# SunBangjie/FYP-BidirectionalPathTracer

Measured on AMD Instinct MI355X. Metric: Mrays/s + RMSE vs the scalar oracle, BDPT pass, Sponza-class scene 1920x1080 depth 8, higher is better.
Workload: dtype f32

## Files before the change

fyp-bidirectionalpathtracer_amd/__init__.py:

```python
import ctypes as C

from . import abi, tiling
from .abi import (Camera, Counters, GBuffer, GBufferParams, Params, SceneDesc, Stripes, Tile, TileInfo, load_library)

__all__ = ["abi", "tiling", "Scene", "Context", "FramePipeline", "load_library", "source_hash", "ADAPTIVE_DEFAULTS",
           "adaptive_params"]

GBUFFER_CHANNELS = ("WorldPosition", "WorldNormal", "MaterialDiffuse", "MaterialSpecRough", "MaterialExtraParams",
                    "Emissive")
OUTPUT_CHANNEL = "PipelineOutput"


class BdptError(RuntimeError):
    pass


def source_hash():
    import glob
    import hashlib
    import os
    here = os.path.dirname(os.path.abspath(__file__))
    root = os.path.dirname(here)
    files = sorted(glob.glob(os.path.join(here, "csrc", "*.hip")) + glob.glob(os.path.join(here, "csrc", "*.hpp")) +
                   glob.glob(os.path.join(here, "csrc", "*.h")) + glob.glob(os.path.join(here, "csrc", "*.cpp")) +
# ... 465 lines not shown
    def sync(self, stream=None):
        self._check(self._lib.bdpt_sync(self._h, stream), "bdpt_sync")

    def test_rng(self, val0, val1, draws):
        import numpy as np
        val0 = np.ascontiguousarray(val0, np.uint32)
        val1 = np.ascontiguousarray(val1, np.uint32)
        n = val0.size
        st = np.zeros((n, draws), np.uint32)
        fl = np.zeros((n, draws), np.float32)
        self._check(self._lib.bdpt_test_rng(self._h, val0.ctypes.data, val1.ctypes.data, n, draws, st.ctypes.data,
                                            fl.ctypes.data), "bdpt_test_rng")
        return st, fl

    def test_trace(self, rays, mode):
        import numpy as np
        rays = np.ascontiguousarray(rays, np.float32).reshape(-1, 8)
        n = rays.shape[0]
        prim = np.zeros(n, np.int32)
        tuv = np.zeros((n, 3), np.float32)
        self._check(self._lib.bdpt_test_trace(self._h, rays.ctypes.data, n, mode, prim.ctypes.data, tuv.ctypes.data),
                    "bdpt_test_trace")
        return prim, tuv

    def test_trace_shadow(self, rays):
        import numpy as np
        rays = np.ascontiguousarray(rays, np.float32)
        n = rays.shape[0]
        vis = np.zeros(n, np.uint8)
        deep = C.c_uint32(0)
        self._check(self._lib.bdpt_test_trace_shadow(self._h, rays.ctypes.data, n, vis.ctypes.data, C.byref(deep)),
                    "bdpt_test_trace_shadow")
        return vis, deep.value

    def test_bsdf(self, recs, mat_index):
        import numpy as np
        recs = np.ascontiguousarray(recs, np.float32).reshape(-1, 20)
        out = np.zeros((recs.shape[0], 16), np.float32)
        self._check(self._lib.bdpt_test_bsdf(self._h, recs.ctypes.data, recs.shape[0], mat_index, out.ctypes.data),
                    "bdpt_test_bsdf")
        return out

    def area_light_info(self):
        info = abi.AreaLightInfo()
        self._check(self._lib.bdpt_get_area_light_info(self._h, C.byref(info)), "bdpt_get_area_light_info")
        return info

    def test_area_light_sample(self, mode, states, points=None):
        import numpy as np
        states = np.ascontiguousarray(states, np.uint32).reshape(-1)
        n = states.shape[0]
        pts = None
        if points is not None:
            pts = np.ascontiguousarray(points, np.float32).reshape(n, 3)
        out = np.zeros((n, 16), np.float32)
        self._check(self._lib.bdpt_test_area_light_sample(self._h, mode, states.ctypes.data,
                                                          None if pts is None else pts.ctypes.data, n, out.ctypes.data),
                    "bdpt_test_area_light_sample")
        return out

    def close(self):
        if self._h:
            self._lib.bdpt_destroy(self._h)
            self._h = None

    def __del__(self):
# ... 217 lines not shown
```

fyp-bidirectionalpathtracer_amd/abi.py:

```python
import ctypes as C
import os

_HERE = os.path.dirname(os.path.abspath(__file__))
LIB_PATH = os.path.join(_HERE, "csrc", "libbdpt_amd.so")

BDPT_MAX_DEPTH = 16
BDPT_MAX_LIGHTS = 16
PARAM_COUNTERS = 1
PARAM_DEFER_RESOLVE = 2
PARAM_NO_NEE = 4
PARAM_NO_SPLAT = 8
PARAM_NO_CONNECT = 16
PARAM_SPECULAR_FROM_LOBE = 32
PARAM_MIS_POWER = 64
PARAM_MIS_LINEAR = 128
PARAM_DEFER_TAIL = 256
PARAM_KEEP_COUNTERS = 512
PARAM_ENV_ON_MISS = 1024
PARAM_EMISSIVE_HITS = 2048
PARAM_AREA_LIGHTS = 4096
PREPARE_PRIMARY = 1
PREPARE_BMFR = 2
PREPARE_REFIT = 4
PREPARE_LIGHT_GROUPS = 8
# ... 195 lines not shown
    "bdpt_adaptive_reset": (C.c_int, [C.c_void_p, C.POINTER(AdaptiveState), C.c_void_p]),
    "bdpt_adaptive_update": (C.c_int, [C.c_void_p, C.POINTER(AdaptiveParams), C.POINTER(AdaptiveState), C.c_void_p, C.c_void_p]),
    "bdpt_prepare": (C.c_int, [C.c_void_p, C.c_uint32]),
    "bdpt_resize_stripes": (C.c_int, [C.c_void_p, C.c_uint32, C.c_uint32, Stripes, C.c_uint32]),
    "bdpt_stripe_rows": (C.c_uint32, [C.c_uint32, C.c_uint32]),
    "bdpt_get_tile_info": (C.c_int, [C.c_void_p, C.POINTER(TileInfo)]),
    "bdpt_tile_row_ranges": (C.c_int, [C.c_void_p, C.POINTER(C.c_uint32), C.c_uint32]),
    "bdpt_resolve_tile": (C.c_int, [C.c_void_p, C.c_void_p, C.c_void_p, C.c_void_p]),
    "bdpt_accumulate_tile": (C.c_int, [C.c_void_p, C.c_void_p, C.c_void_p, C.c_uint32, C.c_uint32, C.c_void_p]),
    "bdpt_test_tree_builder": (C.c_int, [C.c_int]),
    "bdpt_bvh_recs_hash": (C.c_int, [C.POINTER(SceneDesc), C.c_int, C.POINTER(C.c_uint64), C.POINTER(BvhInfo)]),
    "bdpt_bvh_build_hash": (C.c_int, [C.POINTER(SceneDesc), C.c_int, C.POINTER(C.c_uint64), C.POINTER(BvhInfo)]),
    "bdpt_splat_buffer": (C.c_int, [C.c_void_p, C.POINTER(C.c_void_p), C.POINTER(C.c_uint64)]),
    "bdpt_set_splat_buffer": (C.c_int, [C.c_void_p, C.c_void_p, C.c_uint64]),
    "bdpt_resolve": (C.c_int, [C.c_void_p, C.c_void_p, C.c_uint32, C.c_void_p, C.c_void_p]),
    "bdpt_bmfr_execute": (C.c_int, [C.c_void_p, C.POINTER(BmfrParams), C.POINTER(GBuffer), C.c_void_p, C.c_void_p]),
    "bdpt_bmfr_reset": (C.c_int, [C.c_void_p]),
    "bdpt_bmfr_history_bytes": (C.c_int, [C.c_void_p, C.POINTER(C.c_uint64)]),
    "bdpt_bmfr_save_history": (C.c_int, [C.c_void_p, C.c_void_p, C.c_uint64]),
    "bdpt_bmfr_load_history": (C.c_int, [C.c_void_p, C.c_void_p, C.c_uint64]),
    "bdpt_tile_pack": (C.c_int, [C.c_void_p, C.c_void_p, C.c_void_p, C.c_uint32, C.c_void_p]),
    "bdpt_tile_unpack": (C.c_int, [C.c_void_p, C.c_uint32, C.c_void_p, C.c_void_p, C.c_uint32, C.c_void_p]),
    "bdpt_camera_view_proj": (C.c_int, [C.POINTER(C.c_float), C.POINTER(C.c_float), C.POINTER(C.c_float), C.c_float,
                                        C.c_float, C.c_float, C.c_float, C.c_float, C.POINTER(C.c_float)]),
    "bdpt_accumulate": (C.c_int, [C.c_void_p, C.c_void_p, C.c_void_p, C.c_uint32, C.c_uint32, C.c_uint64,
                                  C.c_void_p]),
    "bdpt_get_counters": (C.c_int, [C.c_void_p, C.POINTER(Counters)]),
    "bdpt_get_stage_times": (C.c_int, [C.c_void_p, C.POINTER(C.c_char_p), C.POINTER(C.c_float), C.c_int]),
    "bdpt_enable_stage_timing": (C.c_int, [C.c_void_p, C.c_int]),
    "bdpt_sync": (C.c_int, [C.c_void_p, C.c_void_p]),
    "bdpt_test_rng": (C.c_int, [C.c_void_p, C.c_void_p, C.c_void_p, C.c_uint32, C.c_uint32, C.c_void_p, C.c_void_p]),
    "bdpt_test_trace": (C.c_int, [C.c_void_p, C.c_void_p, C.c_uint32, C.c_int, C.c_void_p, C.c_void_p]),
    "bdpt_test_trace_shadow": (C.c_int, [C.c_void_p, C.c_void_p, C.c_uint32, C.c_void_p, C.c_void_p]),
    "bdpt_test_bsdf": (C.c_int, [C.c_void_p, C.c_void_p, C.c_uint32, C.c_uint32, C.c_void_p]),
    "bdpt_get_area_light_info": (C.c_int, [C.c_void_p, C.POINTER(AreaLightInfo)]),
    "bdpt_test_area_light_sample": (C.c_int, [C.c_void_p, C.c_uint32, C.c_void_p, C.c_void_p, C.c_uint32, C.c_void_p]),
    "bdpt_scene_create_cornell": (C.c_void_p, []),
    "bdpt_scene_create_atrium": (C.c_void_p, [C.c_uint32, C.c_uint32]),
    "bdpt_scene_create_atrium_uneven": (C.c_void_p, [C.c_uint32, C.c_uint32]),
    "bdpt_scene_create_courtyard": (C.c_void_p, [C.c_uint32, C.c_uint32, C.c_float]),
    "bdpt_scene_create_soup": (C.c_void_p, [C.c_uint32, C.c_uint32, C.c_float]),
    "bdpt_scene_load": (C.c_void_p, [C.c_char_p, C.c_char_p, C.c_uint32]),
    "bdpt_scene_load_threads": (C.c_int, [C.c_int]),
    "bdpt_scene_destroy": (None, [C.c_void_p]),
    "bdpt_image_load": (C.c_int, [C.c_char_p, C.POINTER(C.c_uint32), C.POINTER(C.c_uint32), C.POINTER(C.c_uint32), C.c_void_p, C.c_uint64,
                                  C.c_char_p, C.c_uint32]),
    "bdpt_image_load_hdr": (C.c_int, [C.c_char_p, C.POINTER(C.c_uint32), C.POINTER(C.c_uint32), C.c_void_p, C.c_uint64, C.c_char_p, C.c_uint32]),
    "bdpt_scene_get_desc": (C.c_int, [C.c_void_p, C.POINTER(SceneDesc)]),
    "bdpt_scene_get_camera": (C.c_int, [C.c_void_p, C.c_float, C.POINTER(Camera)]),
}

_lib = None


def load_library(path=None):
    global _lib
    if _lib is not None and path is None:
        return _lib
    p = path or LIB_PATH
    if not os.path.exists(p):
        raise RuntimeError(
            f"{p} not found: the HIP extension is not built (run __graft_entry__.build()). "
            "There is no CPU fallback for the render pass.")
    lib = C.CDLL(p, mode=C.RTLD_GLOBAL)
    for name, (res, args) in PROTOTYPES.items():
        fn = getattr(lib, name)
# ... 6 lines not shown
```

fyp-bidirectionalpathtracer_amd/csrc/api.cpp:

```cpp
#include <hip/hip_runtime.h>

#include <cmath>
#include <cstdio>
#include <cstdlib>
#include <cstring>
#include <future>
#include <functional>
#include <atomic>
#include <chrono>
#include <string>
#include <thread>
#include <vector>

#include "../../include/bdpt.h"
#include <new>

#include "bvh.h"
#include "kernels.h"
#include "refit.h"
#include "scene_bvh.h"

using namespace bdpt;

namespace {
// ... 1881 lines not shown
    out_info->numAlwaysPass = sb.numAlwaysPass;
  }
  return BDPT_OK;
} catch (const std::bad_alloc&) {
  return BDPT_E_NOMEM;
} catch (...) {
  return BDPT_E_INVALID;
}

int bdpt_get_counters(bdpt_ctx* c, bdpt_counters* out) {
  if (!c || !out) return BDPT_E_INVALID;
  if (!c->haveSize) return BDPT_E_STATE;
  ENTER(c);
  HIPCHK(c, hipStreamSynchronize(c->lastStream));
  DevCounters h;
  HIPCHK(c, hipMemcpy(&h, c->counters, sizeof(h), hipMemcpyDeviceToHost));
  static_assert(sizeof(bdpt_counters) == 17 * sizeof(uint64_t), "counter fields");
  uint64_t* o = reinterpret_cast<uint64_t*>(out);
  for (int f = 0; f < 13; f++) {
    o[f] = 0;
    for (uint32_t sh = 0; sh < kCounterShards; sh++) o[f] += h.v[sh][f];
  }
  out->alphaTestsClosest = out->alphaTestsShadow = out->hintedNee = out->hintedSplat = 0;
  for (uint32_t sh = 0; sh < kCounterShards; sh++) {
    out->alphaTestsClosest += h.v[sh][C_ALPHA_CLOSEST];
    out->alphaTestsShadow += h.v[sh][C_ALPHA_SHADOW];
    out->hintedNee += h.v[sh][C_HINT_NEE];
    out->hintedSplat += h.v[sh][C_HINT_SPLAT];
  }
  out->raysPrimary = (uint64_t)c->P.Np;
  return BDPT_OK;
}

int bdpt_enable_stage_timing(bdpt_ctx* c, int enable) {
  if (!c) return BDPT_E_INVALID;
  c->timing = enable != 0;
  return BDPT_OK;
}

int bdpt_get_stage_times(bdpt_ctx* c, const char** names, float* ms, int cap) {
  if (!c || !names || !ms) return BDPT_E_INVALID;
  if (!c->timing || c->numStages == 0) return 0;
  ENTER(c);
  HIPCHK(c, hipEventSynchronize(c->ev[c->numStages]));
  int n = std::min(cap, c->numStages);
  for (int i = 0; i < n; i++) {
    names[i] = c->stageNames[i];
    float t = 0.0f;
    HIPCHK(c, hipEventElapsedTime(&t, c->ev[i], c->ev[i + 1]));
    ms[i] = t;
  }
  for (int i = 0; i < c->numSideStages && n < cap; i++, n++) {
    names[n] = c->sideNames[i];
    float t = 0.0f;
    HIPCHK(c, hipEventElapsedTime(&t, c->sideEv[2 * i], c->sideEv[2 * i + 1]));
    ms[n] = t;
  }
  return n;
}

int bdpt_sync(bdpt_ctx* c, void* stream) {
  if (!c) return BDPT_E_INVALID;
  ENTER(c);
  HIPCHK(c, hipStreamSynchronize(reinterpret_cast<hipStream_t>(stream)));
  return BDPT_OK;
}
// ... 173 lines not shown
```

fyp-bidirectionalpathtracer_amd/csrc/device_trace.hpp:

```cpp
#pragma once
#include "bvh.h"
#include "device_scene.hpp"

namespace bdpt {
#define BD __device__ __forceinline__
#define BDPT_ONE_WAVE_PER_GROUP()               \
  do {                                          \
    if (blockDim.x != (unsigned)kWave) return;  \
  } while (0)

struct Hit {
  int prim;
  float t, u, v;
  uint32_t rec;
};

constexpr int kDone = (int)0x80000000;

struct TravState {
  f3 o, d, idir;
  uint32_t neg;
  float tmin, tmax;
  int cur, sp;
  Hit best;
};

BD float clampedRcp(float d) {
  float r = 1.0f / d;
  if (!(fabsf(r) <= 1.0e30f)) r = copysignf(1.0e30f, d);
  return r;
}

BD void travInit(TravState& T, f3 o, f3 d, float tmin, float tmax) {
  T.o = o;
  T.d = d;
  T.idir = mk(clampedRcp(d.x), clampedRcp(d.y), clampedRcp(d.z));
  T.neg = (d.x < 0.0f ? 1u : 0u) | (d.y < 0.0f ? 2u : 0u) | (d.z < 0.0f ? 4u : 0u);
  T.tmin = tmin;
  T.tmax = tmax;
  T.sp = 0;
  T.best.prim = -1;
  T.best.t = tmax;
  T.best.u = 0.0f;
  T.best.v = 0.0f;
  T.best.rec = 0xFFFFFFFFu;
  const bool finite = (o.x == o.x) && (o.y == o.y) && (o.z == o.z) && (d.x == d.x) && (d.y == d.y) && (d.z == d.z);
  T.cur = (finite && (tmax > tmin)) ? 0 : kDone;
}

template <int KL>
BD int* ovfSlot(const SceneDev& S, int e) {
  return S.stackOvf + (size_t)(e - KL) * S.stackOvfStride + (size_t)blockIdx.x * kWave + (threadIdx.x & 63u);
}
template <int KL>
BD void stackStore(const SceneDev& S, int* stk, int e, int ref) {
  if (KL < kStackEntries && e >= KL)
    *ovfSlot<KL>(S, e) = ref;
  else
    stk[e * kWave] = ref;
}
template <int KL>
BD int travPop(const SceneDev& S, TravState& T, const int* stk) {
  if (T.sp == 0) return kDone;
  T.sp--;
  if (KL < kStackEntries && T.sp >= KL) return *ovfSlot<KL>(S, T.sp);
  return stk[T.sp * kWave];
}
template <int KL>
BD void travPush(const SceneDev& S, TravState& T, int* stk, int ref) {
  stackStore<KL>(S, stk, T.sp, ref);
  T.sp++;
}

BD float ubyte(uint32_t w, int c) { return (float)((w >> (8 * c)) & 0xffu); }

template <int ORDER, int KL = kStackEntries>
BD void nodeStep(const SceneDev& S, TravState& T, int* stk) {
  const uint4* np = S.recs + (size_t)T.cur * kRecF4;
  const uint4 q0 = np[0], q1 = np[1], q2 = np[2];
  const float sx = __uint_as_float((q0.w << 23) & 0x7f800000u), sy = __uint_as_float((q0.w << 15) & 0x7f800000u),
              sz = __uint_as_float((q0.w << 7) & 0x7f800000u);
  const float ax = sx * T.idir.x, ay = sy * T.idir.y, az = sz * T.idir.z;
  const float bx = (__uint_as_float(q0.x) - T.o.x) * T.idir.x, by = (__uint_as_float(q0.y) - T.o.y) * T.idir.y,
              bz = (__uint_as_float(q0.z) - T.o.z) * T.idir.z;
// ... 388 lines not shown
```

fyp-bidirectionalpathtracer_amd/csrc/kernels.h:

```cpp
#pragma once
#include <hip/hip_runtime.h>
#include <stdint.h>

#include "../../include/bdpt.h"
#include "texture_planes.h"

namespace bdpt {

constexpr int kWave = 64;
#ifndef KSTACK
#define KSTACK 32
#endif
constexpr int kStackEntries = KSTACK;
#ifndef BDPT_STACK_LDS
#define BDPT_STACK_LDS 24
#endif
constexpr int kStackLds = BDPT_STACK_LDS < KSTACK ? BDPT_STACK_LDS : KSTACK;
constexpr int kMaxPersistentPerCU = 32;
constexpr int kStackOvfRows = KSTACK - kStackLds;
constexpr int kShadeRecF4 = 7;
constexpr uint32_t kNoRay = 0xFFFFFFFFu;
constexpr uint32_t kNumSubQueues = 32;
#ifndef BDPT_FETCH_CHUNK
#define BDPT_FETCH_CHUNK 256
#endif
constexpr uint32_t kFetchChunk = BDPT_FETCH_CHUNK;
constexpr uint32_t kCursorStride = 32;
constexpr uint32_t kCursorBlock = kNumSubQueues * kCursorStride;
#ifndef BDPT_RAY_SUBQUEUES
#define BDPT_RAY_SUBQUEUES 32
#endif
constexpr uint32_t kNumRaySubQueues = BDPT_RAY_SUBQUEUES;
constexpr uint32_t kRayCursorBlock = kNumRaySubQueues * kCursorStride;
constexpr uint32_t kCounterShards = 64;

enum : int { F_COL = 0, F_POS = 3, F_N = 6, F_V = 9, F_DIF = 12, F_SPEC = 15, F_ROUGH = 18, F_ISSPEC = 19, F_PDF = 20, NF = 21 };
constexpr int NF4 = 6;
enum : int { PATH_EYE = 0, PATH_LIGHT = 1 };
enum : int { RAY_TERMS = 0, RAY_PAIRS = 1 };

struct TexDev {
  const uint8_t* px;
  uint32_t w, h, srgb, pow2;
};

struct SceneConst {
  bdpt_light lights[BDPT_MAX_LIGHTS];
  float srgbLut[256];
};

struct SceneDev {
  const uint4* recs;
  const float4* shade;
  const float* bitangents;
  const uint32_t* indices;
  const bdpt_material* materials;
  const TexDev* textures;
  const TexDev* matTex;
  const SceneConst* sc;
  uint32_t numLights;
  uint32_t hasBitangents;
  uint32_t numRecs;
  const float4* alphaRecs;
  int* stackOvf;
  uint32_t stackOvfStride;
  const uint32_t* lightMap;
  uint32_t lightMapRes;
};

struct DevCounters {
  unsigned long long v[kCounterShards][32];
};
enum : int {
  C_RAYS_PRIMARY = 0, C_RAYS_EYE, C_RAYS_LIGHT, C_RAYS_NEE, C_RAYS_SPLAT, C_RAYS_CONNECT,
  C_NODE_CLOSEST, C_TRI_CLOSEST, C_NODE_SHADOW, C_TRI_SHADOW, C_PIX_VALID, C_SPLATS, C_RAYS_LAZY,
  C_STACK_MAX,
  C_ALPHA_CLOSEST, C_ALPHA_SHADOW,
  C_HINT_NEE, C_HINT_SPLAT
};

inline __host__ __device__ uint32_t numConnectPairs(uint32_t D) {
  uint32_t n = 0;
  for (uint32_t t = 2; t <= D; t++) n += (t < D - 1) ? t : (D - 1);
  return n;
}

struct PathBuf {
  float* v;
  float* rayDir;
  const uint32_t* pix;
  uint32_t* seedE;
  uint32_t* seedL;
  uint8_t* eyeLast;
  uint8_t* lightLast;
  uint8_t* lightReal;
  uint32_t* queue[3];
  uint32_t pathSubCap;
  uint32_t* qcount;
  uint32_t* qhead;
  float* rayQ;
  float* rayContrib;
  uint8_t* rayVis;
  uint32_t* rayCount;
  uint32_t* rayHead;
  uint32_t raySubCap[2];
  uint32_t rayBase[2];
  uint32_t* slotRay;
  uint32_t* splatPix;
  float* misE;
  float* misL;
  uint8_t* lazyCursor;
// ... 158 lines not shown
```

fyp-bidirectionalpathtracer_amd/csrc/kernels.hip:

```cpp
#include "kernels.h"

#include <algorithm>
#include <type_traits>

#include "device_area.hpp"
#include "device_math.hpp"
#include "device_scene.hpp"
#include "device_trace.hpp"
#include "launch.hpp"

namespace bdpt {

#define BD __device__ __forceinline__

BD void wavePush(bool active, uint32_t value, uint32_t* items, uint32_t* count, uint32_t subCap, uint32_t q = 0xffffffffu) {
  unsigned long long mask = __ballot(active);
  if (mask == 0ull) return;
  const int lane = (int)(threadIdx.x & 63u);
  const int leader = __ffsll((long long)mask) - 1;
  if (q == 0xffffffffu) q = blockIdx.x % kNumSubQueues;
  uint32_t base = 0;
  if (lane == leader) base = atomicAdd(&count[q * kCursorStride], (uint32_t)__popcll(mask));
  base = (uint32_t)__shfl((int)base, leader);
  const uint32_t prefix = (uint32_t)__popcll(mask & ((1ull << lane) - 1ull));
// ... 311 lines not shown
  BDPT_ONE_WAVE_PER_GROUP();
  initPathsLane<GGX, V == FrameKind::Groups, V == FrameKind::Masked>(S, F, P, groupOf(A), maskOf(A));
}
template <bool GGX, FrameKind V>
__global__ __launch_bounds__(kWave) void init_paths_area_kernel(SceneDev S, FrameDev F, PathBuf P, FrameArg<V> A, AreaDev E) {
  BDPT_ONE_WAVE_PER_GROUP();
  initPathsLane<GGX, false, V == FrameKind::Masked, true>(S, F, P, GroupDev{}, maskOf(A), E);
}

constexpr uint32_t kPoolEntries = 128;
#ifndef BDPT_WALK_ORDER
#define BDPT_WALK_ORDER 1
#endif
#ifndef BDPT_WALK_SHADE_MIN
#define BDPT_WALK_SHADE_MIN 64
#endif
#ifndef BDPT_WALK_LEAF_WAIT
#define BDPT_WALK_LEAF_WAIT 1
#endif
#ifndef BDPT_WALK_NODE_BURST
#define BDPT_WALK_NODE_BURST 3
#endif
#ifndef BDPT_WALK_CHUNK
#define BDPT_WALK_CHUNK 64
#endif
#ifndef BDPT_WALK_REFILL
#define BDPT_WALK_REFILL BDPT_REFILL_IDLE
#endif
BD uint32_t packPath(uint32_t p, int path, int k) { return p | ((uint32_t)path << 24) | ((uint32_t)k << 25); }

#ifndef BDPT_WALK_WAVES_PER_EU
#define BDPT_WALK_WAVES_PER_EU 4
#endif
#ifndef BDPT_WALK_STACK_LDS
#define BDPT_WALK_STACK_LDS kStackEntries
#endif
constexpr int kWalkStackLds = BDPT_WALK_STACK_LDS;
constexpr uint32_t kParkedMiss = 1u << 30;
template <bool GGX, bool COUNT, bool EXT, bool MASKED>
__global__ __launch_bounds__(kWave) __attribute__((amdgpu_waves_per_eu(BDPT_WALK_WAVES_PER_EU, 8))) void walk_kernel(
    SceneDev S, FrameDev F, PathBuf P, uint32_t* __restrict__ head, FrameArg<MASKED ? FrameKind::Masked : FrameKind::Plain> mask) {
  BDPT_ONE_WAVE_PER_GROUP();
  __shared__ int s_stack[kWalkStackLds * kWave];
  __shared__ uint4 s_pool[kPoolEntries];
  const MaskDev& M = maskOf(mask);
  int* stk = s_stack + threadIdx.x;
  const int lane = (int)(threadIdx.x & 63u);
  const unsigned long long laneBelow = (1ull << lane) - 1ull;
  const int D = (int)F.p.maxDepth;
  const bool fromLobe = (F.p.flags & BDPT_PARAM_SPECULAR_FROM_LOBE) != 0;
  const uint32_t firstV = (D >= 2) ? 0u : kNumSubQueues, numV = 2u * kNumSubQueues - firstV;
  bool trav = false;
  uint32_t id = 0;
  TravState T;
  travInit(T, mk(0), mk(0), F.p.minT, 1.0e38f);
  T.cur = kDone;
  uint32_t nNodes = 0, nTris = 0, nAlpha = 0;
  uint32_t nEye = 0, nLight = 0, nParked = 0, nReady = 0;
  uint32_t vq = firstV + blockIdx.x % numV, tried = 0, chunkPos = 0, chunkEnd = 0, chunk = BDPT_WALK_CHUNK;
  bool exhausted = false;
  const uint32_t wavesPerList = (gridDim.x + numV - 1) / numV;
  for (;;) {
    unsigned long long travMask = __ballot(trav);
    const bool flush = (travMask == 0ull) && nReady == 0 && exhausted && nParked > 0;
    if (nParked >= (uint32_t)BDPT_WALK_SHADE_MIN || flush) {
      const uint32_t n = nParked < (uint32_t)kWave ? nParked : (uint32_t)kWave;
      nParked -= n;
      const bool act = (uint32_t)lane < n;
      uint4 rec = make_uint4(0, 0, 0, 0);
      if (act) rec = s_pool[nParked + (uint32_t)lane];
      __syncthreads();
      const uint32_t p = rec.x & 0xffffffu;
      const int path = (int)((rec.x >> 24) & 1u), k = (int)((rec.x >> 25) & 31u);
      nEye += (uint32_t)__popcll(__ballot(act && path == PATH_EYE));
      nLight += (uint32_t)__popcll(__ballot(act && path == PATH_LIGHT));
      bool survive = false;
      f3 L = mk(0);
      if (act) {
        const bool miss = EXT ? (rec.x & kParkedMiss) != 0u : (int)rec.y < 0;
        const int prim = miss ? -1 : (int)rec.y;
        const f3 o = ldPlane3(P, path, k, F_POS, p);
        f3 found = mk(0);
        bool haveFound = false;
        if (prim >= 0) {
          const uint32_t seed = (path == PATH_EYE) ? P.seedE[p] : P.seedL[p];
          const f3 thr = ldPlane3(P, path, k, F_COL, p);
          Shading sd = shadeHit<false>(S, (uint32_t)prim, __uint_as_float(rec.z), __uint_as_float(rec.w), o);
          float pdf;
          bool isSpec;
          f3 w = sampleBRDF<GGX>(seed, sd.N, sd.N, sd.V, sd.diffuse, sd.specular, sd.roughness, fromLobe, L, pdf, isSpec);
          Vtx v;
          v.color = thr * w;
          v.pos = sd.posW;
          v.N = sd.N;
          v.V = sd.V;
          v.dif = sd.diffuse;
          v.spec = sd.specular;
          v.rough = sd.roughness;
          v.isSpec = isSpec;
          v.pdf = pdf;
          storeVtx(P, path, k + 1, p, v);
          survive = (k + 2 <= D);
          if (EXT && path == PATH_EYE && (F.p.flags & BDPT_PARAM_EMISSIVE_HITS) &&
              (sd.emissive.x > 0.0f || sd.emissive.y > 0.0f || sd.emissive.z > 0.0f)) {
            found = thr * sd.emissive;
            haveFound = true;
          }
        } else {
          if (EXT && path == PATH_EYE && (F.p.flags & BDPT_PARAM_ENV_ON_MISS)) {
            const f3 dir = mk(__uint_as_float(rec.y), __uint_as_float(rec.z), __uint_as_float(rec.w));
            const f3 env = F.envMap ? envLookup(F.envMap, F.envW, F.envH, dir) : ld3(F.envColor);
            found = ldPlane3(P, path, k, F_COL, p) * env;
            haveFound = true;
          }
          Vtx g = zeroVtx();
          if (path == PATH_EYE && k == 1) {
            g.pos = o;
          } else {
            loadSurf(P, path, k, p, g);
            g.V = ldPlane3(P, path, k, F_V, p);
            if (path == PATH_LIGHT && k == 0) g.pdf = 0.0f;
          }
          g.color = mk(0);
          storeVtx(P, path, k + 1, p, g);
          if (path == PATH_EYE) {
            P.eyeLast[p] = (uint8_t)(k + 1);
          } else {
            P.lightLast[p] = (uint8_t)(k + 1);
            P.lightReal[p] = (uint8_t)k;
          }
        }
        if (MASKED && haveFound && M.mask[P.pix[p]] == 0) haveFound = false;
        if (EXT && haveFound) {
          f3 term = clampVec(found / (float)(k + 1), F.p.clampUpper);
          if (isnan3(term)) term = mk(0);
          float4* out4 = reinterpret_cast<float4*>(F.out);
          const size_t pix = P.pix[p];
          float4 acc = out4[pix];
          acc.x = acc.x + term.x;
          acc.y = acc.y + term.y;
          acc.z = acc.z + term.z;
          acc.w = acc.w + 1.0f;
          out4[pix] = acc;
        }
      }
      const unsigned long long sm = __ballot(survive);
      if (survive) {
        const uint32_t slot = kPoolEntries - 1u - nReady - (uint32_t)__popcll(sm & laneBelow);
        s_pool[slot] = make_uint4(packPath(p, path, k + 1), __float_as_uint(L.x), __float_as_uint(L.y), __float_as_uint(L.z));
      }
      nReady += (uint32_t)__popcll(sm);
      __builtin_amdgcn_fence(__ATOMIC_RELEASE, "workgroup");
      __syncthreads();
    }
    const int empty = 64 - __popcll(travMask);
    if ((empty >= BDPT_WALK_REFILL || travMask == 0ull) && (nReady > 0 || !exhausted)) {
      const unsigned long long emptyMask = ~travMask;
      const uint32_t rank = (uint32_t)__popcll(emptyMask & laneBelow);
      const uint32_t fromReady = ((uint32_t)empty < nReady) ? (uint32_t)empty : nReady;
      bool got = false;
      uint32_t nid = 0;
      f3 dir = mk(0);
      if (!trav && rank < fromReady) {
        const uint4 r = s_pool[kPoolEntries - nReady + rank];
        nid = r.x;
        dir = mk(__uint_as_float(r.y), __uint_as_float(r.z), __uint_as_float(r.w));
        got = true;
      }
      __syncthreads();
      nReady -= fromReady;
      uint32_t want = (uint32_t)empty - fromReady;
      uint32_t taken = fromReady;
      while (want > 0 && !exhausted) {
        while (chunkPos >= chunkEnd && !exhausted) {
          const uint32_t* counts = (MASKED && vq < kNumSubQueues) ? M.walkEyeCount : P.qcount;
          const uint32_t nq = counts[(vq % kNumSubQueues) * kCursorStride];
          uint32_t base = nq;
          if (__hip_atomic_load(&head[vq * kCursorStride], __ATOMIC_RELAXED, __HIP_MEMORY_SCOPE_AGENT) < nq) {
            uint32_t share = (nq / wavesPerList + 15u) & ~15u;
            chunk = share < 16u ? 16u : (share > (uint32_t)BDPT_WALK_CHUNK ? (uint32_t)BDPT_WALK_CHUNK : share);
            if (lane == 0) base = atomicAdd(&head[vq * kCursorStride], chunk);
            base = (uint32_t)__builtin_amdgcn_readfirstlane((int)base);
          }
          if (base < nq) {
            chunkPos = base;
            chunkEnd = (base + chunk < nq) ? base + chunk : nq;
            tried = 0;
          } else {
            vq = (vq + 1 == 2u * kNumSubQueues) ? firstV : vq + 1;
            if (++tried >= numV) exhausted = true;
          }
        }
        if (exhausted) break;
        const uint32_t avail = chunkEnd - chunkPos;
        const uint32_t take = (want < avail) ? want : avail;
        if (!trav && !got && rank >= taken && rank < taken + take) {
          const uint32_t* items = (MASKED && vq < kNumSubQueues) ? M.walkEye : P.queue[0];
          const uint32_t p = items[(vq % kNumSubQueues) * P.pathSubCap + chunkPos + (rank - taken)];
          const int path = (int)(vq / kNumSubQueues);
          const float* rd = P.rayDir + (size_t)(path * 3) * P.Np + p;
          nid = packPath(p, path, (path == PATH_EYE) ? 1 : 0);
          dir = mk(rd[0], rd[P.Np], rd[2 * (size_t)P.Np]);
          got = true;
        }
        chunkPos += take;
        taken += take;
        want -= take;
      }
      if (got) {
        id = nid;
        travInit(T, ldPlane3(P, (int)((nid >> 24) & 1u), (int)(nid >> 25), F_POS, nid & 0xffffffu), dir, F.p.minT, 1.0e38f);
        trav = true;
      }
      travMask = __ballot(trav);
    }
    if (travMask == 0ull) {
      if (nParked == 0 && nReady == 0 && exhausted) break;
      continue;
    }
    bool finished = false;
#if BDPT_WALK_LEAF_WAIT > 0
    if (trav) {
#pragma unroll 1
      for (int kk = 0; kk < BDPT_WALK_NODE_BURST && T.cur >= 0; kk++) {
        if (COUNT) nNodes++;
        nodeStep<BDPT_WALK_ORDER, kWalkStackLds>(S, T, stk);
      }
    }
    {
      const unsigned long long waitMask = __ballot(trav && T.cur < 0), nodeMask = __ballot(trav && T.cur >= 0);
      const int waitNeed = (__popcll(waitMask | nodeMask) * BDPT_LEAF_WAIT_FRAC8 + 7) >> 3;
      if ((int)__popcll(waitMask) >= waitNeed || nodeMask == 0ull) {
        if (trav && T.cur < 0) {
          finished = (T.cur == kDone);
          if (!finished) {
            finished = leafStep<0, COUNT>(S, T, nTris, nAlpha);
            if (!finished) {
              T.cur = travPop<kWalkStackLds>(S, T, stk);
              finished = (T.cur == kDone);
            }
          }
        }
      }
    }
#else
    if (trav) {
      while (T.cur >= 0) {
        if (COUNT) nNodes++;
        nodeStep<BDPT_WALK_ORDER, kWalkStackLds>(S, T, stk);
      }
      finished = (T.cur == kDone);
      if (!finished) {
        finished = leafStep<0, COUNT>(S, T, nTris, nAlpha);
        if (!finished) {
          T.cur = travPop<kWalkStackLds>(S, T, stk);
          finished = (T.cur == kDone);
        }
      }
    }
#endif
    const unsigned long long finMask = __ballot(finished);
    if (finMask) {
      if (finished) {
        const bool miss = T.best.prim < 0;
        s_pool[nParked + (uint32_t)__popcll(finMask & laneBelow)] =
            (EXT && miss) ? make_uint4(id | kParkedMiss, __float_as_uint(T.d.x), __float_as_uint(T.d.y), __float_as_uint(T.d.z))
                          : make_uint4(id, (uint32_t)T.best.prim, __float_as_uint(T.best.u), __float_as_uint(T.best.v));
        trav = false;
      }
      nParked += (uint32_t)__popcll(finMask);
      __syncthreads();
    }
  }
  if (lane == 0) {
    if (nEye) atomicAdd(&F.counters->v[blockIdx.x % kCounterShards][C_RAYS_EYE], (unsigned long long)nEye);
    if (nLight) atomicAdd(&F.counters->v[blockIdx.x % kCounterShards][C_RAYS_LIGHT], (unsigned long long)nLight);
  }
  if (COUNT) {
    waveAddCount(F.counters, C_NODE_CLOSEST, nNodes);
    waveAddCount(F.counters, C_TRI_CLOSEST, nTris);
    waveAddCount(F.counters, C_ALPHA_CLOSEST, nAlpha);
  }
}

BD float evalGWithoutVPos(f3 posA, f3 nA, f3 posB, f3 nB) {
  const f3 vecAB = posB - posA;
  const float invLengthAB = 1.0f / length(vecAB);
  const f3 dirAB = vecAB * invLengthAB;
  const float cosA = fabsf(dot(nA, dirAB));
  const float cosB = fabsf(dot(nB, dirAB));
  return cosA * cosB * invLengthAB * invLengthAB;
}

__global__ __launch_bounds__(kWave) void mis_prefix_kernel(FrameDev F, PathBuf P) {
  BDPT_ONE_WAVE_PER_GROUP();
  bool act = false;
  uint32_t i = 0;
  if (!queueChunk(P.qcount, P.pathSubCap, act, i)) return;
  if (!act) return;
  const uint32_t p = P.queue[0][i];
  const int D = (int)F.p.maxDepth;
  const int eyeLast = P.eyeLast[p], lightLast = P.lightLast[p];
  f3 prevPos = ld3(F.cam.posW), prevN = normalize(ld3(F.cam.cameraW));
  float pE = 1.0f;
  P.misE[p] = pE;
  for (int x = 1; x <= D; x++) {
    f3 pos = mk(0), N = mk(0);
    float pdf = 0.0f;
    if (x <= eyeLast) {
      pos = ldPlane3(P, PATH_EYE, x, F_POS, p);
      N = ldPlane3(P, PATH_EYE, x, F_N, p);
      pdf = ldPlane1(P, PATH_EYE, x, F_PDF, p);
    }
    pE *= pdf * evalGWithoutVPos(prevPos, prevN, pos, N);
// ... 1096 lines not shown
```

include/bdpt.h:

```cpp
#ifndef BDPT_H_
#define BDPT_H_

#include <stdint.h>

#ifdef __cplusplus
extern "C" {
#endif

#define BDPT_OK 0
#define BDPT_E_INVALID (-1)
#define BDPT_E_STATE (-2)
#define BDPT_E_HIP (-3)
#define BDPT_E_NOMEM (-4)
#define BDPT_E_LIMIT (-5)

#define BDPT_MAX_LIGHTS 16
#define BDPT_MAX_DEPTH 16

#define BDPT_LIGHT_POINT 0
#define BDPT_LIGHT_DIRECTIONAL 1

#define BDPT_SHADING_MODEL_METAL_ROUGH 0u
#define BDPT_SHADING_MODEL_SPEC_GLOSS 2u
#define BDPT_CHANNEL_UNUSED 0u
// ... 377 lines not shown
int bdpt_bmfr_execute(bdpt_ctx* ctx, const bdpt_bmfr_params* p, const bdpt_gbuffer* features, float* noisy, void* stream);

int bdpt_bmfr_reset(bdpt_ctx* ctx);

int bdpt_bmfr_history_bytes(const bdpt_ctx* ctx, uint64_t* out_bytes);
int bdpt_bmfr_save_history(bdpt_ctx* ctx, void* host_blob, uint64_t bytes);
int bdpt_bmfr_load_history(bdpt_ctx* ctx, const void* host_blob, uint64_t bytes);

int bdpt_tile_pack(bdpt_ctx* ctx, const void* frame, void* packed, uint32_t bytesPerPixel, void* stream);
int bdpt_tile_unpack(bdpt_ctx* ctx, uint32_t owner, const void* packed, void* frame, uint32_t bytesPerPixel, void* stream);

int bdpt_camera_view_proj(const float pos[3], const float target[3], const float up[3], float focalLengthMm,
                          float frameHeightMm, float aspect, float nearZ, float farZ, float out16[16]);

int bdpt_get_counters(bdpt_ctx* ctx, bdpt_counters* out);

int bdpt_get_stage_times(bdpt_ctx* ctx, const char** names, float* ms, int cap);
int bdpt_enable_stage_timing(bdpt_ctx* ctx, int enable);

int bdpt_sync(bdpt_ctx* ctx, void* stream);

typedef struct bdpt_area_light_info {
  uint32_t numEmitters;
  uint32_t numTextured;
  float totalWeight;
  uint32_t reserved;
} bdpt_area_light_info;
int bdpt_get_area_light_info(bdpt_ctx* ctx, bdpt_area_light_info* out);

int bdpt_test_rng(bdpt_ctx* ctx, const uint32_t* val0, const uint32_t* val1, uint32_t n, uint32_t draws,
                  uint32_t* out_states, float* out_floats);
int bdpt_test_trace(bdpt_ctx* ctx, const float* rays, uint32_t n, int mode, int32_t* out_prim, float* out_tuv);
int bdpt_test_trace_shadow(bdpt_ctx* ctx, const float* rays, uint32_t n, uint8_t* out_vis, uint32_t* out_max_stack);
int bdpt_test_bsdf(bdpt_ctx* ctx, const float* in, uint32_t n, uint32_t matIndex, float* out);
int bdpt_test_area_light_sample(bdpt_ctx* ctx, uint32_t mode, const uint32_t* states, const float* points, uint32_t n, float* out);

#ifdef __cplusplus
}
#endif
#endif
```

Before: 4814.

## Carry ray origin and throughput through LDS pool in walk kernel

The walk kernel now keeps each parked ray's origin and throughput in a new LDS side pool, and the in-flight ray id and throughput in a per-lane LDS array. The shade step reads these from LDS instead of reloading vertex position and color planes from global memory, and the traversal restart reads them from LDS too. It also drops some barriers and a release fence, shrinks the walk traversal stack kept in LDS from the full stack depth to 16 rows (deeper entries spill to the global overflow buffer), and adds a counter plus test API for the walk stack's maximum depth. The cost is extra LDS per workgroup, which may lower occupancy, and more overflow traffic when traversal goes deep.

Result: faster. 5012, median of 6 (+4.1%).

```diff
diff --git a/fyp-bidirectionalpathtracer_amd/__init__.py b/fyp-bidirectionalpathtracer_amd/__init__.py
--- a/fyp-bidirectionalpathtracer_amd/__init__.py
+++ b/fyp-bidirectionalpathtracer_amd/__init__.py
@@ -521,6 +521,11 @@
         self._check(self._lib.bdpt_test_trace_shadow(self._h, rays.ctypes.data, n, vis.ctypes.data, C.byref(deep)),
                     "bdpt_test_trace_shadow")
         return vis, deep.value
+
+    def test_walk_stack(self):
+        deep, rows = C.c_uint32(0), C.c_uint32(0)
+        self._check(self._lib.bdpt_test_walk_stack(self._h, C.byref(deep), C.byref(rows)), "bdpt_test_walk_stack")
+        return deep.value, rows.value
 
     def test_bsdf(self, recs, mat_index):
         import numpy as np
diff --git a/fyp-bidirectionalpathtracer_amd/abi.py b/fyp-bidirectionalpathtracer_amd/abi.py
--- a/fyp-bidirectionalpathtracer_amd/abi.py
+++ b/fyp-bidirectionalpathtracer_amd/abi.py
@@ -251,6 +251,7 @@
     "bdpt_test_rng": (C.c_int, [C.c_void_p, C.c_void_p, C.c_void_p, C.c_uint32, C.c_uint32, C.c_void_p, C.c_void_p]),
     "bdpt_test_trace": (C.c_int, [C.c_void_p, C.c_void_p, C.c_uint32, C.c_int, C.c_void_p, C.c_void_p]),
     "bdpt_test_trace_shadow": (C.c_int, [C.c_void_p, C.c_void_p, C.c_uint32, C.c_void_p, C.c_void_p]),
+    "bdpt_test_walk_stack": (C.c_int, [C.c_void_p, C.c_void_p, C.c_void_p]),
     "bdpt_test_bsdf": (C.c_int, [C.c_void_p, C.c_void_p, C.c_uint32, C.c_uint32, C.c_void_p]),
     "bdpt_get_area_light_info": (C.c_int, [C.c_void_p, C.POINTER(AreaLightInfo)]),
     "bdpt_test_area_light_sample": (C.c_int, [C.c_void_p, C.c_uint32, C.c_void_p, C.c_void_p, C.c_uint32, C.c_void_p]),
diff --git a/fyp-bidirectionalpathtracer_amd/csrc/api.cpp b/fyp-bidirectionalpathtracer_amd/csrc/api.cpp
--- a/fyp-bidirectionalpathtracer_amd/csrc/api.cpp
+++ b/fyp-bidirectionalpathtracer_amd/csrc/api.cpp
@@ -1937,6 +1937,20 @@
   return BDPT_OK;
 }
 
+int bdpt_test_walk_stack(bdpt_ctx* c, uint32_t* out_max_stack, uint32_t* out_lds_rows) {
+  if (!c) return BDPT_E_INVALID;
+  if (!c->haveSize) return BDPT_E_STATE;
+  ENTER(c);
+  HIPCHK(c, hipStreamSynchronize(c->lastStream));
+  DevCounters h;
+  HIPCHK(c, hipMemcpy(&h, c->counters, sizeof(h), hipMemcpyDeviceToHost));
+  unsigned long long m = 0;
+  for (uint32_t sh = 0; sh < kCounterShards; sh++) m = std::max(m, h.v[sh][C_STACK_MAX_WALK]);
+  if (out_max_stack) *out_max_stack = (uint32_t)m;
+  if (out_lds_rows) *out_lds_rows = (uint32_t)kWalkStackLds;
+  return BDPT_OK;
+}
+
 int bdpt_enable_stage_timing(bdpt_ctx* c, int enable) {
   if (!c) return BDPT_E_INVALID;
   c->timing = enable != 0;
diff --git a/fyp-bidirectionalpathtracer_amd/csrc/device_trace.hpp b/fyp-bidirectionalpathtracer_amd/csrc/device_trace.hpp
--- a/fyp-bidirectionalpathtracer_amd/csrc/device_trace.hpp
+++ b/fyp-bidirectionalpathtracer_amd/csrc/device_trace.hpp
@@ -50,6 +50,7 @@
 
 template <int KL>
 BD int* ovfSlot(const SceneDev& S, int e) {
+  if (KL < kStackLds) return S.stackOvf + ((uint32_t)(e - KL) * S.stackOvfStride + blockIdx.x * (uint32_t)kWave + (threadIdx.x & 63u));
   return S.stackOvf + (size_t)(e - KL) * S.stackOvfStride + (size_t)blockIdx.x * kWave + (threadIdx.x & 63u);
 }
 template <int KL>
diff --git a/fyp-bidirectionalpathtracer_amd/csrc/kernels.h b/fyp-bidirectionalpathtracer_amd/csrc/kernels.h
--- a/fyp-bidirectionalpathtracer_amd/csrc/kernels.h
+++ b/fyp-bidirectionalpathtracer_amd/csrc/kernels.h
@@ -16,8 +16,12 @@
 #define BDPT_STACK_LDS 24
 #endif
 constexpr int kStackLds = BDPT_STACK_LDS < KSTACK ? BDPT_STACK_LDS : KSTACK;
+#ifndef BDPT_WALK_STACK_LDS
+#define BDPT_WALK_STACK_LDS 16
+#endif
+constexpr int kWalkStackLds = BDPT_WALK_STACK_LDS < KSTACK ? BDPT_WALK_STACK_LDS : KSTACK;
 constexpr int kMaxPersistentPerCU = 32;
-constexpr int kStackOvfRows = KSTACK - kStackLds;
+constexpr int kStackOvfRows = KSTACK - (kWalkStackLds < kStackLds ? kWalkStackLds : kStackLds);
 constexpr int kShadeRecF4 = 7;
 constexpr uint32_t kNoRay = 0xFFFFFFFFu;
 constexpr uint32_t kNumSubQueues = 32;
@@ -76,7 +80,8 @@
   C_NODE_CLOSEST, C_TRI_CLOSEST, C_NODE_SHADOW, C_TRI_SHADOW, C_PIX_VALID, C_SPLATS, C_RAYS_LAZY,
   C_STACK_MAX,
   C_ALPHA_CLOSEST, C_ALPHA_SHADOW,
-  C_HINT_NEE, C_HINT_SPLAT
+  C_HINT_NEE, C_HINT_SPLAT,
+  C_STACK_MAX_WALK
 };
 
 inline __host__ __device__ uint32_t numConnectPairs(uint32_t D) {
diff --git a/fyp-bidirectionalpathtracer_amd/csrc/kernels.hip b/fyp-bidirectionalpathtracer_amd/csrc/kernels.hip
--- a/fyp-bidirectionalpathtracer_amd/csrc/kernels.hip
+++ b/fyp-bidirectionalpathtracer_amd/csrc/kernels.hip
@@ -367,17 +367,33 @@
 #ifndef BDPT_WALK_WAVES_PER_EU
 #define BDPT_WALK_WAVES_PER_EU 4
 #endif
-#ifndef BDPT_WALK_STACK_LDS
-#define BDPT_WALK_STACK_LDS kStackEntries
-#endif
-constexpr int kWalkStackLds = BDPT_WALK_STACK_LDS;
 constexpr uint32_t kParkedMiss = 1u << 30;
+BD void poolStore2(uint2 (*pl)[kPoolEntries], uint32_t slot, f3 o, f3 thr) {
+  pl[0][slot] = make_uint2(__float_as_uint(o.x), __float_as_uint(o.y));
+  pl[1][slot] = make_uint2(__float_as_uint(o.z), __float_as_uint(thr.x));
+  pl[2][slot] = make_uint2(__float_as_uint(thr.y), __float_as_uint(thr.z));
+}
+BD f3 poolLoadOrigin(const uint2 (*pl)[kPoolEntries], uint32_t slot) {
+  const uint2 a = pl[0][slot];
+  return mk(__uint_as_float(a.x), __uint_as_float(a.y), __uint_as_float(pl[1][slot].x));
+}
+BD f3 poolLoadThr(const uint2 (*pl)[kPoolEntries], uint32_t slot) {
+  const uint2 c = pl[2][slot];
+  return mk(__uint_as_float(pl[1][slot].y), __uint_as_float(c.x), __uint_as_float(c.y));
+}
+BD void poolLoad2(const uint2 (*pl)[kPoolEntries], uint32_t slot, f3& o, f3& thr) {
+  const uint2 a = pl[0][slot], b = pl[1][slot], c = pl[2][slot];
+  o = mk(__uint_as_float(a.x), __uint_as_float(a.y), __uint_as_float(b.x));
+  thr = mk(__uint_as_float(b.y), __uint_as_float(c.x), __uint_as_float(c.y));
+}
 template <bool GGX, bool COUNT, bool EXT, bool MASKED>
 __global__ __launch_bounds__(kWave) __attribute__((amdgpu_waves_per_eu(BDPT_WALK_WAVES_PER_EU, 8))) void walk_kernel(
     SceneDev S, FrameDev F, PathBuf P, uint32_t* __restrict__ head, FrameArg<MASKED ? FrameKind::Masked : FrameKind::Plain> mask) {
   BDPT_ONE_WAVE_PER_GROUP();
   __shared__ int s_stack[kWalkStackLds * kWave];
   __shared__ uint4 s_pool[kPoolEntries];
+  __shared__ uint2 s_pool2[3][kPoolEntries];
+  __shared__ uint32_t s_ray[4 * kWave];
   const MaskDev& M = maskOf(mask);
   int* stk = s_stack + threadIdx.x;
   const int lane = (int)(threadIdx.x & 63u);
@@ -386,11 +402,11 @@
   const bool fromLobe = (F.p.flags & BDPT_PARAM_SPECULAR_FROM_LOBE) != 0;
   const uint32_t firstV = (D >= 2) ? 0u : kNumSubQueues, numV = 2u * kNumSubQueues - firstV;
   bool trav = false;
-  uint32_t id = 0;
   TravState T;
   travInit(T, mk(0), mk(0), F.p.minT, 1.0e38f);
   T.cur = kDone;
   uint32_t nNodes = 0, nTris = 0, nAlpha = 0;
+  int maxSp = 0;
   uint32_t nEye = 0, nLight = 0, nParked = 0, nReady = 0;
   uint32_t vq = firstV + blockIdx.x % numV, tried = 0, chunkPos = 0, chunkEnd = 0, chunk = BDPT_WALK_CHUNK;
   bool exhausted = false;
@@ -403,27 +419,30 @@
       nParked -= n;
       const bool act = (uint32_t)lane < n;
       uint4 rec = make_uint4(0, 0, 0, 0);
-      if (act) rec = s_pool[nParked + (uint32_t)lane];
-      __syncthreads();
+      f3 o = mk(0);
+      const uint32_t recSlot = nParked + (uint32_t)lane;
+      if (act) {
+        rec = s_pool[recSlot];
+        o = poolLoadOrigin(s_pool2, recSlot);
+      }
       const uint32_t p = rec.x & 0xffffffu;
       const int path = (int)((rec.x >> 24) & 1u), k = (int)((rec.x >> 25) & 31u);
       nEye += (uint32_t)__popcll(__ballot(act && path == PATH_EYE));
       nLight += (uint32_t)__popcll(__ballot(act && path == PATH_LIGHT));
       bool survive = false;
-      f3 L = mk(0);
+      f3 L = mk(0), nextO = mk(0), nextThr = mk(0);
+      f3 found = mk(0);
+      bool haveFound = false;
+      const bool miss = act && (EXT ? (rec.x & kParkedMiss) != 0u : (int)rec.y < 0);
       if (act) {
-        const bool miss = EXT ? (rec.x & kParkedMiss) != 0u : (int)rec.y < 0;
         const int prim = miss ? -1 : (int)rec.y;
-        const f3 o = ldPlane3(P, path, k, F_POS, p);
-        f3 found = mk(0);
-        bool haveFound = false;
         if (prim >= 0) {
           const uint32_t seed = (path == PATH_EYE) ? P.seedE[p] : P.seedL[p];
-          const f3 thr = ldPlane3(P, path, k, F_COL, p);
           Shading sd = shadeHit<false>(S, (uint32_t)prim, __uint_as_float(rec.z), __uint_as_float(rec.w), o);
           float pdf;
           bool isSpec;
           f3 w = sampleBRDF<GGX>(seed, sd.N, sd.N, sd.V, sd.diffuse, sd.specular, sd.roughness, fromLobe, L, pdf, isSpec);
+          const f3 thr = poolLoadThr(s_pool2, recSlot);
           Vtx v;
           v.color = thr * w;
           v.pos = sd.posW;
@@ -436,16 +455,20 @@
           v.pdf = pdf;
           storeVtx(P, path, k + 1, p, v);
           survive = (k + 2 <= D);
+          nextO = v.pos;
+          nextThr = v.color;
           if (EXT && path == PATH_EYE && (F.p.flags & BDPT_PARAM_EMISSIVE_HITS) &&
               (sd.emissive.x > 0.0f || sd.emissive.y > 0.0f || sd.emissive.z > 0.0f)) {
-            found = thr * sd.emissive;
+            found = poolLoadThr(s_pool2, recSlot) * sd.emissive;
             haveFound = true;
           }
         } else {
           if (EXT && path == PATH_EYE && (F.p.flags & BDPT_PARAM_ENV_ON_MISS)) {
             const f3 dir = mk(__uint_as_float(rec.y), __uint_as_float(rec.z), __uint_as_float(rec.w));
-            const f3 env = F.envMap ? envLookup(F.envMap, F.envW, F.envH, dir) : ld3(F.envColor);
-            found = ldPlane3(P, path, k, F_COL, p) * env;
+            uint32_t envW = F.envW, envH = F.envH;
+            asm volatile("" : "+s"(envW), "+s"(envH));
+            const f3 env = F.envMap ? envLookup(F.envMap, envW, envH, dir) : ld3(F.envColor);
+            found = poolLoadThr(s_pool2, recSlot) * env;
             haveFound = true;
           }
           Vtx g = zeroVtx();
@@ -466,7 +489,16 @@
           }
         }
         if (MASKED && haveFound && M.mask[P.pix[p]] == 0) haveFound = false;
-        if (EXT && haveFound) {
+      }
+      __syncthreads();
+      const unsigned long long sm = __ballot(survive);
+      if (survive) {
+        const uint32_t slot = kPoolEntries - 1u - nReady - (uint32_t)__popcll(sm & laneBelow);
+        s_pool[slot] = make_uint4(packPath(p, path, k + 1), __float_as_uint(L.x), __float_as_uint(L.y), __float_as_uint(L.z));
+        poolStore2(s_pool2, slot, nextO, nextThr);
+      }
+      if (EXT) {
+        if (haveFound) {
           f3 term = clampVec(found / (float)(k + 1), F.p.clampUpper);
           if (isnan3(term)) term = mk(0);
           float4* out4 = reinterpret_cast<float4*>(F.out);
@@ -479,13 +511,7 @@
           out4[pix] = acc;
         }
       }
-      const unsigned long long sm = __ballot(survive);
-      if (survive) {
-        const uint32_t slot = kPoolEntries - 1u - nReady - (uint32_t)__popcll(sm & laneBelow);
-        s_pool[slot] = make_uint4(packPath(p, path, k + 1), __float_as_uint(L.x), __float_as_uint(L.y), __float_as_uint(L.z));
-      }
       nReady += (uint32_t)__popcll(sm);
-      __builtin_amdgcn_fence(__ATOMIC_RELEASE, "workgroup");
       __syncthreads();
     }
     const int empty = 64 - __popcll(travMask);
@@ -493,16 +519,13 @@
       const unsigned long long emptyMask = ~travMask;
       const uint32_t rank = (uint32_t)__popcll(emptyMask & laneBelow);
       const uint32_t fromReady = ((uint32_t)empty < nReady) ? (uint32_t)empty : nReady;
-      bool got = false;
+      bool got = false, fresh = false;
       uint32_t nid = 0;
       f3 dir = mk(0);
       if (!trav && rank < fromReady) {
-        const uint4 r = s_pool[kPoolEntries - nReady + rank];
-        nid = r.x;
-        dir = mk(__uint_as_float(r.y), __uint_as_float(r.z), __uint_as_float(r.w));
+        nid = kPoolEntries - nReady + rank;
         got = true;
       }
-      __syncthreads();
       nReady -= fromReady;
       uint32_t want = (uint32_t)empty - fromReady;
       uint32_t taken = fromReady;
@@ -536,17 +559,33 @@
           const float* rd = P.rayDir + (size_t)(path * 3) * P.Np + p;
           nid = packPath(p, path, (path == PATH_EYE) ? 1 : 0);
           dir = mk(rd[0], rd[P.Np], rd[2 * (size_t)P.Np]);
-          got = true;
+          got = fresh = true;
         }
         chunkPos += take;
         taken += take;
         want -= take;
       }
       if (got) {
-        id = nid;
-        travInit(T, ldPlane3(P, (int)((nid >> 24) & 1u), (int)(nid >> 25), F_POS, nid & 0xffffffu), dir, F.p.minT, 1.0e38f);
+        f3 org, thr;
+        if (fresh) {
+          const float4* r = vtxPtr(P, (int)((nid >> 24) & 1u), (int)(nid >> 25), nid & 0xffffffu);
+          const float4 q0 = r[fieldQ(F_POS)], q4 = r[fieldQ(F_COL)];
+          org = mk(q0.x, q0.y, q0.z);
+          thr = mk(q4.x, q4.y, q4.z);
+        } else {
+          const uint4 r = s_pool[nid];
+          poolLoad2(s_pool2, nid, org, thr);
+          nid = r.x;
+          dir = mk(__uint_as_float(r.y), __uint_as_float(r.z), __uint_as_float(r.w));
+        }
+        travInit(T, org, dir, F.p.minT, 1.0e38f);
+        s_ray[lane] = nid;
+        s_ray[kWave + lane] = __float_as_uint(thr.x);
+        s_ray[2 * kWave + lane] = __float_as_uint(thr.y);
+        s_ray[3 * kWave + lane] = __float_as_uint(thr.z);
         trav = true;
       }
+      __syncthreads();
       travMask = __ballot(trav);
     }
     if (travMask == 0ull) {
@@ -554,12 +593,14 @@
       continue;
     }
     bool finished = false;
+    int roundSp = 0;
 #if BDPT_WALK_LEAF_WAIT > 0
     if (trav) {
 #pragma unroll 1
       for (int kk = 0; kk < BDPT_WALK_NODE_BURST && T.cur >= 0; kk++) {
         if (COUNT) nNodes++;
         nodeStep<BDPT_WALK_ORDER, kWalkStackLds>(S, T, stk);
+        if (COUNT) roundSp = T.sp > roundSp ? T.sp : roundSp;
       }
     }
     {
@@ -583,6 +624,7 @@
       while (T.cur >= 0) {
         if (COUNT) nNodes++;
         nodeStep<BDPT_WALK_ORDER, kWalkStackLds>(S, T, stk);
+        if (COUNT) roundSp = T.sp > roundSp ? T.sp : roundSp;
       }
       finished = (T.cur == kDone);
       if (!finished) {
@@ -594,11 +636,18 @@
       }
     }
 #endif
+    if (COUNT) {
+      while (__ballot(roundSp > maxSp) != 0ull) maxSp++;
+    }
     const unsigned long long finMask = __ballot(finished);
     if (finMask) {
       if (finished) {
         const bool miss = T.best.prim < 0;
-        s_pool[nParked + (uint32_t)__popcll(finMask & laneBelow)] =
+        const uint32_t slot = nParked + (uint32_t)__popcll(finMask & laneBelow);
+        const uint32_t id = s_ray[lane];
+        poolStore2(s_pool2, slot, T.o,
+                   mk(__uint_as_float(s_ray[kWave + lane]), __uint_as_float(s_ray[2 * kWave + lane]), __uint_as_float(s_ray[3 * kWave + lane])));
+        s_pool[slot] =
             (EXT && miss) ? make_uint4(id | kParkedMiss, __float_as_uint(T.d.x), __float_as_uint(T.d.y), __float_as_uint(T.d.z))
                           : make_uint4(id, (uint32_t)T.best.prim, __float_as_uint(T.best.u), __float_as_uint(T.best.v));
         trav = false;
@@ -615,6 +664,7 @@
     waveAddCount(F.counters, C_NODE_CLOSEST, nNodes);
     waveAddCount(F.counters, C_TRI_CLOSEST, nTris);
     waveAddCount(F.counters, C_ALPHA_CLOSEST, nAlpha);
+    if (maxSp > 0 && lane == 0) atomicMax(&F.counters->v[blockIdx.x % kCounterShards][C_STACK_MAX_WALK], (unsigned long long)maxSp);
   }
 }
 
diff --git a/include/bdpt.h b/include/bdpt.h
--- a/include/bdpt.h
+++ b/include/bdpt.h
@@ -433,6 +433,7 @@
                   uint32_t* out_states, float* out_floats);
 int bdpt_test_trace(bdpt_ctx* ctx, const float* rays, uint32_t n, int mode, int32_t* out_prim, float* out_tuv);
 int bdpt_test_trace_shadow(bdpt_ctx* ctx, const float* rays, uint32_t n, uint8_t* out_vis, uint32_t* out_max_stack);
+int bdpt_test_walk_stack(bdpt_ctx* ctx, uint32_t* out_max_stack, uint32_t* out_lds_rows);
 int bdpt_test_bsdf(bdpt_ctx* ctx, const float* in, uint32_t n, uint32_t matIndex, float* out);
 int bdpt_test_area_light_sample(bdpt_ctx* ctx, uint32_t mode, const uint32_t* states, const float* points, uint32_t n, float* out);
 
```
